# FangjinhuaWang/PatchmatchNet

Measured on AMD Instinct MI355X. Metric: depth-maps/sec at 1600x1200 N=5 src views, higher is better.
Workload: dtype f32

## Files before the change

patchmatchnet_amd/csrc/aggregate.hip:

```cpp
#include <cstring>

#include "pmn_common.hpp"
#define PMN_DIV_DM1(acc, D) ((acc) / (float)((D) - 1))

struct AggArgs {
    const float* cost;
    const float* depth;
    const float* xnorm;
    const float* fweight;
    const float* offsets;
    float* score;
    float* depth_out;
    int K, is_inverse, B, D, h, w;
    float interval_scale;
    int table[2 * PMN_MAX_NEIGHBORS];
};

template <int KMAX, int DL>
__global__ __launch_bounds__(PMN_BLOCK, (KMAX <= 9 ? 3 : 1)) void aggregate_regress_kernel(const AggArgs a) {
#pragma clang fp contract(off)
    constexpr int NPX = PMN_BLOCK / DL;
    __shared__ float red[DL][NPX];
    __shared__ float red2[DL][NPX];
    const int h = a.h, w = a.w, hw = h * w, D = a.D, K = a.K;
// ... 73 lines not shown

    float acc = 0.0f;
#pragma unroll 1
    for (int d = dl; d < D; d += DL) {
        if (ok) {
            const size_t o = ((size_t)b * D + d) * hw + p;
            const float prob = expf((a.score[o] - smax) - lse);
            a.score[o] = prob;
            acc = acc + (a.is_inverse ? (float)d : a.depth[o]) * prob;
        }
    }
    red2[dl][px] = acc;
    __syncthreads();
    if (dl != 0 || !ok) return;
    acc = 0.0f;
#pragma unroll
    for (int i = 0; i < DL; ++i) acc = acc + red2[i][px];
    float out = acc;
    if (a.is_inverse) {
        const float inv_min = 1.0f / a.depth[((size_t)b * D + (D - 1)) * hw + p];
        const float inv_max = 1.0f / a.depth[((size_t)b * D) * hw + p];
        const float inv = inv_max + PMN_DIV_DM1(acc, D) * (inv_min - inv_max);
        out = 1.0f / inv;
    }
    a.depth_out[(size_t)b * hw + p] = out;
}

__device__ __forceinline__ float sigmoid_rcp(float x) {
    const float d = 1.0f + __builtin_amdgcn_exp2f(x * -1.4426950408889634f);
    float r = __builtin_amdgcn_rcpf(d);
    return r * fmaf(-d, r, 2.0f);
}

template <int G, int SL>
__device__ __forceinline__ int agg_group_bcast_i(int v) {
    static_assert(G == 2 || G == 4 || G == 8 || G == 16, "lane groups inside a DPP row");
    if constexpr (G == 2) {
        return __builtin_amdgcn_mov_dpp(v, SL | (SL << 2) | ((2 + SL) << 4) | ((2 + SL) << 6), 0xF, 0xF, true);
    } else if constexpr (G == 4) {
        return __builtin_amdgcn_mov_dpp(v, SL | (SL << 2) | (SL << 4) | (SL << 6), 0xF, 0xF, true);
    } else if constexpr (G == 16) {
        return __builtin_amdgcn_mov_dpp(v, 0x150 + SL, 0xF, 0xF, true);
    } else {
        const int lo = __builtin_amdgcn_update_dpp(v, v, 0x150 + SL, 0xF, 0x3, false);
        return __builtin_amdgcn_update_dpp(lo, v, 0x150 + 8 + SL, 0xF, 0xC, false);
    }
}
template <int G, int SL>
__device__ __forceinline__ float agg_group_bcast_f(float v) {
    return __int_as_float(agg_group_bcast_i<G, SL>(__float_as_int(v)));
}

template <int KMAX>
__device__ __forceinline__ void agg_form_tap_set(const AggArgs& a, int b, int k, int p, int x, int y, int& off, float& w00, float& w01,
                                                 float& w10, float& w11, float& fw) {
    const int h = a.h, w = a.w, hw = h * w, K = a.K;
    const float ox = a.offsets[((size_t)b * 2 * K + 2 * k) * hw + p];
    const float oy = a.offsets[((size_t)b * 2 * K + 2 * k + 1) * hw + p];
    float ix, iy;
    pmn_neighbor_position((float)x, (float)y, a.table[2 * k], a.table[2 * k + 1], ox, oy, h, w, ix, iy);
    const PmnTaps t = pmn_make_taps(ix, iy, h, w);
    off = t.off;
    w00 = t.w00;
    w01 = t.w01;
    w10 = t.w10;
    w11 = t.w11;
    fw = a.fweight[((size_t)b * K + k) * hw + p];
}

template <int KMAX, int DQT>
__global__ __launch_bounds__(PMN_BLOCK, (KMAX <= 9 ? 3 : 1)) void aggregate_regress_q4_kernel(const AggArgs a) {
#pragma clang fp contract(off)
    __shared__ float red[PMN_BLOCK];
    const int h = a.h, w = a.w, hw = h * w, D = a.D, K = a.K, DQ = DQT > 0 ? DQT : D >> 2;
    const int npx = blockDim.x / DQ;
    const int px = threadIdx.x / DQ, q = threadIdx.x - px * DQ;
    const int p_raw = blockIdx.x * npx + px;
    const bool ok = p_raw < hw;
    const int p = ok ? p_raw : hw - 1;
    const int b = blockIdx.y;
    const int y = p / w, x = p - y * w;

    int off[KMAX];
    float w00[KMAX], w01[KMAX], w10[KMAX], w11[KMAX], fw[KMAX];
    if constexpr (DQT > 1) {
        constexpr int KPT = (KMAX + DQT - 1) / DQT;
        int moff[KPT];
        float m00[KPT], m01[KPT], m10[KPT], m11[KPT], mfw[KPT];
#pragma unroll
        for (int i = 0; i < KPT; ++i) {
            const int k = q + i * DQT;
            moff[i] = 0;
            m00[i] = m01[i] = m10[i] = m11[i] = mfw[i] = 0.0f;
            if (k < K) agg_form_tap_set<KMAX>(a, b, k, p, x, y, moff[i], m00[i], m01[i], m10[i], m11[i], mfw[i]);
        }
#define AGG_TAKE(k_)                                                                                         \
    if constexpr ((k_) < KMAX) {                                                                               \
        constexpr int sl_ = (k_) % DQT, it_ = (k_) / DQT;                                                      \
        off[k_] = agg_group_bcast_i<DQT, sl_>(moff[it_]);                                                      \
        w00[k_] = agg_group_bcast_f<DQT, sl_>(m00[it_]);                                                       \
        w01[k_] = agg_group_bcast_f<DQT, sl_>(m01[it_]);                                                       \
        w10[k_] = agg_group_bcast_f<DQT, sl_>(m10[it_]);                                                       \
        w11[k_] = agg_group_bcast_f<DQT, sl_>(m11[it_]);                                                       \
        fw[k_] = agg_group_bcast_f<DQT, sl_>(mfw[it_]);                                                        \
    }
        AGG_TAKE(0) AGG_TAKE(1) AGG_TAKE(2) AGG_TAKE(3) AGG_TAKE(4) AGG_TAKE(5) AGG_TAKE(6) AGG_TAKE(7) AGG_TAKE(8)
        static_assert(KMAX <= 9, "AGG_TAKE list");
#undef AGG_TAKE
    } else {
#pragma unroll
        for (int k = 0; k < KMAX; ++k) {
            off[k] = 0;
            w00[k] = w01[k] = w10[k] = w11[k] = fw[k] = 0.0f;
            if (k < K) agg_form_tap_set<KMAX>(a, b, k, p, x, y, off[k], w00[k], w01[k], w10[k], w11[k], fw[k]);
        }
    }

    const float inv_interval = 1.0f / a.interval_scale;
    const float* xn = a.xnorm + (size_t)b * hw * D + 4 * q;
    const float* cs = a.cost + (size_t)b * hw * D + 4 * q;
    const float4 xc4 = *reinterpret_cast<const float4*>(xn + (size_t)p * D);
    const float xc[4] = {xc4.x, xc4.y, xc4.z, xc4.w};
    float wk[KMAX][4], ck[KMAX][4], wsum[4] = {0.f, 0.f, 0.f, 0.f};
#pragma unroll
    for (int k = 0; k < KMAX; ++k) {
#pragma unroll
        for (int j = 0; j < 4; ++j) wk[k][j] = ck[k][j] = 0.0f;
        if (k < K) {
            const size_t o = (size_t)off[k] * D, o2 = o + (size_t)w * D;
            const float4 xa = *reinterpret_cast<const float4*>(xn + o), xb = *reinterpret_cast<const float4*>(xn + o + D);
            const float4 xcn = *reinterpret_cast<const float4*>(xn + o2), xd = *reinterpret_cast<const float4*>(xn + o2 + D);
            const float4 ca = *reinterpret_cast<const float4*>(cs + o), cb = *reinterpret_cast<const float4*>(cs + o + D);
            const float4 cc = *reinterpret_cast<const float4*>(cs + o2), cd = *reinterpret_cast<const float4*>(cs + o2 + D);
            const float x00[4] = {xa.x, xa.y, xa.z, xa.w}, x01[4] = {xb.x, xb.y, xb.z, xb.w};
            const float x10[4] = {xcn.x, xcn.y, xcn.z, xcn.w}, x11[4] = {xd.x, xd.y, xd.z, xd.w};
            const float c00[4] = {ca.x, ca.y, ca.z, ca.w}, c01[4] = {cb.x, cb.y, cb.z, cb.w};
            const float c10[4] = {cc.x, cc.y, cc.z, cc.w}, c11[4] = {cd.x, cd.y, cd.z, cd.w};
#pragma unroll
            for (int j = 0; j < 4; ++j) {
                const float x1 = fmaf(x11[j], w11[k], fmaf(x10[j], w10[k], fmaf(x01[j], w01[k], x00[j] * w00[k])));
                ck[k][j] = fmaf(c11[j], w11[k], fmaf(c10[j], w10[k], fmaf(c01[j], w01[k], c00[j] * w00[k])));
                float t = fabsf(x1 - xc[j]) * inv_interval;
                t = fminf(fmaxf(t, 0.0f), 4.0f);
                wk[k][j] = sigmoid_rcp(4.0f - 2.0f * t) * fw[k];
                wsum[j] = wsum[j] + wk[k][j];
            }
        }
    }
    float s[4] = {0.f, 0.f, 0.f, 0.f}, rsum[4];
#pragma unroll
    for (int j = 0; j < 4; ++j) rsum[j] = 1.0f / wsum[j];
#pragma unroll
    for (int k = 0; k < KMAX; ++k)
        if (k < K) {
#pragma unroll
            for (int j = 0; j < 4; ++j) s[j] = s[j] + ck[k][j] * (wk[k][j] * rsum[j]);
        }

    float smax = fmaxf(fmaxf(s[0], s[1]), fmaxf(s[2], s[3]));
    red[threadIdx.x] = smax;
    __syncthreads();
    for (int i = 0; i < DQ; ++i) smax = fmaxf(smax, red[px * DQ + i]);
    __syncthreads();
    float esum = ((expf(s[0] - smax) + expf(s[1] - smax)) + expf(s[2] - smax)) + expf(s[3] - smax);
    red[threadIdx.x] = esum;
    __syncthreads();
    esum = 0.0f;
    for (int i = 0; i < DQ; ++i) esum = esum + red[px * DQ + i];
    __syncthreads();
    const float lse = logf(esum);
    float acc = 0.0f;
#pragma unroll
    for (int j = 0; j < 4; ++j) {
        const int d = 4 * q + j;
        const size_t o = ((size_t)b * D + d) * hw + p;
        const float prob = expf((s[j] - smax) - lse);
        if (ok) a.score[o] = prob;
        acc = acc + (a.is_inverse ? (float)d : a.depth[o]) * prob;
    }
    red[threadIdx.x] = acc;
    __syncthreads();
    if (q != 0 || !ok) return;
    acc = 0.0f;
    for (int i = 0; i < DQ; ++i) acc = acc + red[px * DQ + i];
    float out = acc;
    if (a.is_inverse) {
        const float inv_min = 1.0f / a.depth[((size_t)b * D + (D - 1)) * hw + p];
        const float inv_max = 1.0f / a.depth[((size_t)b * D) * hw + p];
        const float inv = inv_max + PMN_DIV_DM1(acc, D) * (inv_min - inv_max);
        out = 1.0f / inv;
    }
    a.depth_out[(size_t)b * hw + p] = out;
}

template <int KMAX>
static int launch_agg_q4(const AggArgs& a, hipStream_t s) {
    const int DQ = a.D / 4, npx = PMN_BLOCK / DQ;
    const dim3 grid((a.h * a.w + npx - 1) / npx, a.B), block(npx * DQ);
    if (DQ == 2) PMN_LAUNCH((aggregate_regress_q4_kernel<KMAX, 2>), grid, block, 0, s, a);
    else if (DQ == 4) PMN_LAUNCH((aggregate_regress_q4_kernel<KMAX, 4>), grid, block, 0, s, a);
    else if (DQ == 8) PMN_LAUNCH((aggregate_regress_q4_kernel<KMAX, 8>), grid, block, 0, s, a);
    else if (DQ == 16) PMN_LAUNCH((aggregate_regress_q4_kernel<KMAX, 16>), grid, block, 0, s, a);
    else PMN_LAUNCH((aggregate_regress_q4_kernel<KMAX, 0>), grid, block, 0, s, a);
    PMN_CHECK_LAUNCH();
    return PMN_OK;
}

template <int KMAX, int DL>
static int launch_agg_dl(const AggArgs& a, hipStream_t s) {
    constexpr int NPX = PMN_BLOCK / DL;
    const dim3 grid((a.h * a.w + NPX - 1) / NPX, a.B), block(PMN_BLOCK);
    PMN_LAUNCH((aggregate_regress_kernel<KMAX, DL>), grid, block, 0, s, a);
    PMN_CHECK_LAUNCH();
    return PMN_OK;
}

template <int KMAX>
static int launch_agg(const AggArgs& a, hipStream_t s) {
    if constexpr (KMAX <= 9) {
        if (a.D % 4 == 0) return launch_agg_q4<KMAX>(a, s);
    }
    if (a.D >= 32) return launch_agg_dl<KMAX, 16>(a, s);
    if (a.D >= 16) return launch_agg_dl<KMAX, 4>(a, s);
    return launch_agg_dl<KMAX, 1>(a, s);
}

extern "C" int pmn_aggregate_regress(const float* cost, const float* depth_sample, const float* xnorm,
                                     const float* feature_weight, const float* eval_offsets, const int* eval_table_host,
                                     int K, float interval_scale, int is_inverse, int B, int D, int h, int w,
                                     float* score_out, float* depth_out, void* stream) {
    if (!cost || !depth_sample || !xnorm || !feature_weight || !eval_offsets || !eval_table_host || !score_out ||
        !depth_out)
        return PMN_ERR_ARG;
    if (B < 1 || D < 1 || h < 2 || w < 2) return PMN_ERR_ARG;
    if (K < 1 || K > PMN_MAX_NEIGHBORS || D > PMN_MAX_DEPTH) return PMN_ERR_SHAPE;
    if (is_inverse && D < 2) return PMN_ERR_ARG;
    AggArgs a;
    memset(&a, 0, sizeof(a));
    a.cost = cost;
    a.depth = depth_sample;
    a.xnorm = xnorm;
    a.fweight = feature_weight;
    a.offsets = eval_offsets;
    a.score = score_out;
    a.depth_out = depth_out;
    a.K = K;
    a.is_inverse = is_inverse;
    a.B = B; a.D = D; a.h = h; a.w = w;
    a.interval_scale = interval_scale;
    for (int i = 0; i < 2 * K; ++i) a.table[i] = eval_table_host[i];
    if (K <= 9) return launch_agg<9>(a, (hipStream_t)stream);
    return launch_agg<17>(a, (hipStream_t)stream);
}
```

patchmatchnet_amd/csrc/hypotheses.hip:

```cpp
#include <cstring>

#include "pmn_common.hpp"
#define PMN_DIV48(u) ((u) / 48.0f)
#define PMN_DIV48R(u) pmn_div_by((u), 48.0f, r48)

struct HypArgs {
    const float* noise;
    const float* depth;
    const float* depth_min;
    const float* depth_max;
    const float* offsets;
    float* depth_sample;
    float* xnorm;
    int depth_shift, num_sample, K, B, h, w;
    float interval_scale;
    int table[2 * PMN_MAX_NEIGHBORS];
};

__device__ __forceinline__ float centre_hypothesis(const HypArgs& a, int b, int qy, int qx, float inv_min, float inv_max,
                                                   float interval, int kc) {
#pragma clang fp contract(off)
    const int h = a.h, w = a.w;
    if (a.noise) {
        const float u = a.noise[((size_t)b * 48 + 24) * h * w + (size_t)qy * w + qx] + 24.0f;
// ... 79 lines not shown
#pragma unroll
        for (int kk = 2; kk <= NP2; kk <<= 1) {
#pragma unroll
            for (int jj = kk >> 1; jj > 0; jj >>= 1) {
#pragma unroll
                for (int i = 0; i < NP2; ++i) {
                    const int l = i ^ jj;
                    if (l > i) {
                        const float lo = fminf(v[i], v[l]), hi = fmaxf(v[i], v[l]);
                        if ((i & kk) == 0) {
                            v[i] = lo;
                            v[l] = hi;
                        } else {
                            v[i] = hi;
                            v[l] = lo;
                        }
                    }
                }
            }
        }
    }

    const float range = inv_min - inv_max;
#pragma unroll
    for (int j = 0; j < NP2; ++j) {
        if (j < D) {
            const size_t o = ((size_t)b * D + j) * hw + p;
            a.depth_sample[o] = v[j];
            a.xnorm[((size_t)b * hw + p) * D + j] = (1.0f / v[j] - inv_max) / range;
        }
    }
}

template <int NP2, int D0T, int KT>
__global__ __launch_bounds__(PMN_BLOCK) void init_hypotheses_fixed_kernel(const HypArgs a) {
#pragma clang fp contract(off)
    static_assert(D0T + KT <= NP2, "hypotheses fit the sorting network");
    const int h = a.h, w = a.w, hw = h * w;
    const int p = blockIdx.x * blockDim.x + threadIdx.x;
    const int b = blockIdx.y;
    if (p >= hw) return;
    const int y = p / w, x = p - y * w;
    const float inv_min = 1.0f / a.depth_min[b];
    const float inv_max = 1.0f / a.depth_max[b];
    constexpr int D = D0T + KT;
    const float interval = (inv_min - inv_max) * a.interval_scale;
    const int k0 = -((a.num_sample + 1) / 2);
    const int kc = k0 + a.num_sample / 2;
    const bool from_noise = a.noise != nullptr;
    const float r48 = pmn_uniform(pmn_rcp_refined(48.0f));

    float v[NP2];
#pragma unroll
    for (int j = 0; j < NP2; ++j) v[j] = __builtin_inff();

    const int ws = w >> a.depth_shift;
    if (from_noise) {
        float u[D0T];
#pragma unroll
        for (int j = 0; j < D0T; ++j) u[j] = a.noise[((size_t)b * 48 + j) * hw + p];
#pragma unroll
        for (int j = 0; j < D0T; ++j) {
            const float inv = inv_max + PMN_DIV48R(u[j] + (float)j) * (inv_min - inv_max);
            v[j] = pmn_div(1.0f, inv);
        }
    } else {
        const float dprev =
            a.depth[(size_t)b * (h >> a.depth_shift) * ws + (size_t)(y >> a.depth_shift) * ws + (x >> a.depth_shift)];
        if (D0T == 1) {
            v[0] = dprev;
        } else {
            const float inv_prev = pmn_div(1.0f, dprev);
#pragma unroll
            for (int j = 0; j < D0T; ++j) {
                float inv = inv_prev + interval * (float)(k0 + j);
                inv = fminf(fmaxf(inv, inv_max), inv_min);
                v[j] = pmn_div(1.0f, inv);
            }
        }
    }

    if constexpr (KT > 0) {
        constexpr int KB = KT < 8 ? KT : 8;
        static_assert(KT % KB == 0, "whole batches");
        const float* cbase = from_noise ? a.noise + ((size_t)b * 48 + 24) * hw
                                        : a.depth + (size_t)b * (h >> a.depth_shift) * ws;
        const int sh = from_noise ? 0 : a.depth_shift, cw = from_noise ? w : ws;
#pragma unroll
        for (int k0b = 0; k0b < KT; k0b += KB) {
            float ox[KB], oy[KB];
#pragma unroll
            for (int i = 0; i < KB; ++i) {
                ox[i] = a.offsets[((size_t)b * 2 * KT + 2 * (k0b + i)) * hw + p];
                oy[i] = a.offsets[((size_t)b * 2 * KT + 2 * (k0b + i) + 1) * hw + p];
            }
            PmnTaps t[KB];
            float c[KB][4];
#pragma unroll
            for (int i = 0; i < KB; ++i) {
                float ix, iy;
                pmn_neighbor_position((float)x, (float)y, a.table[2 * (k0b + i)], a.table[2 * (k0b + i) + 1], ox[i], oy[i], h, w, ix,
                                      iy);
                t[i] = pmn_make_taps(ix, iy, h, w);
                const int qy = t[i].off / w, qx = t[i].off - qy * w;
                c[i][0] = cbase[(size_t)(qy >> sh) * cw + (qx >> sh)];
                c[i][1] = cbase[(size_t)(qy >> sh) * cw + ((qx + 1) >> sh)];
                c[i][2] = cbase[(size_t)((qy + 1) >> sh) * cw + (qx >> sh)];
                c[i][3] = cbase[(size_t)((qy + 1) >> sh) * cw + ((qx + 1) >> sh)];
            }
#pragma unroll
            for (int i = 0; i < KB; ++i) {
                float cc[4];
#pragma unroll
                for (int q = 0; q < 4; ++q) {
                    if (from_noise) {
                        const float inv = inv_max + PMN_DIV48R(c[i][q] + 24.0f) * (inv_min - inv_max);
                        cc[q] = pmn_div(1.0f, inv);
                    } else if (a.num_sample == 1) {
                        cc[q] = c[i][q];
                    } else {
                        float inv = pmn_div(1.0f, c[i][q]) + interval * (float)kc;
                        inv = fminf(fmaxf(inv, inv_max), inv_min);
                        cc[q] = pmn_div(1.0f, inv);
                    }
                }
                v[D0T + k0b + i] = fmaf(cc[3], t[i].w11, fmaf(cc[2], t[i].w10, fmaf(cc[1], t[i].w01, cc[0] * t[i].w00)));
            }
        }
#pragma unroll
        for (int kk = 2; kk <= NP2; kk <<= 1) {
#pragma unroll
            for (int jj = kk >> 1; jj > 0; jj >>= 1) {
#pragma unroll
                for (int i = 0; i < NP2; ++i) {
                    const int l = i ^ jj;
                    if (l > i) {
                        const float lo = fminf(v[i], v[l]), hi = fmaxf(v[i], v[l]);
                        if ((i & kk) == 0) {
                            v[i] = lo;
                            v[l] = hi;
                        } else {
                            v[i] = hi;
                            v[l] = lo;
                        }
                    }
                }
            }
        }
    }

    const float range = inv_min - inv_max, rrange = pmn_rcp_refined(range);
#pragma unroll
    for (int j = 0; j < D; ++j) {
        const size_t o = ((size_t)b * D + j) * hw + p;
        a.depth_sample[o] = v[j];
        a.xnorm[((size_t)b * hw + p) * D + j] = pmn_div_by(pmn_div(1.0f, v[j]) - inv_max, range, rrange);
    }
}

extern "C" int pmn_init_hypotheses(const float* noise, const float* depth, int depth_shift, const float* depth_min,
                                   const float* depth_max, int num_sample, float interval_scale,
                                   const float* propa_offsets, const int* propa_table_host, int K, int B, int h, int w,
                                   float* depth_sample, float* xnorm, void* stream) {
    if ((!noise && !depth) || !depth_min || !depth_max || !depth_sample || !xnorm) return PMN_ERR_ARG;
    if (B < 1 || h < 2 || w < 2 || K < 0 || depth_shift < 0 || depth_shift > 1) return PMN_ERR_ARG;
    if (K > 0 && (!propa_offsets || !propa_table_host)) return PMN_ERR_ARG;
    if (K > 16) return PMN_ERR_SHAPE;
    if (!noise && num_sample < 1) return PMN_ERR_ARG;
    if (depth_shift && ((h | w) & 1)) return PMN_ERR_ARG;
    const int D0 = noise ? 48 : num_sample;
    const int D = D0 + K;
    if (D > PMN_MAX_DEPTH) return PMN_ERR_SHAPE;
    HypArgs a;
    memset(&a, 0, sizeof(a));
    a.noise = noise;
    a.depth = noise ? nullptr : depth;
    a.depth_min = depth_min;
    a.depth_max = depth_max;
    a.offsets = propa_offsets;
    a.depth_sample = depth_sample;
    a.xnorm = xnorm;
    a.depth_shift = depth_shift;
    a.num_sample = noise ? 48 : num_sample;
    a.K = K;
    a.B = B; a.h = h; a.w = w;
    a.interval_scale = interval_scale;
    for (int i = 0; i < 2 * K; ++i) a.table[i] = propa_table_host[i];
    const int bs = (h * w <= 64 * 1024) ? 64 : PMN_BLOCK;
    const dim3 grid((h * w + bs - 1) / bs, B), block(bs);
    hipStream_t s = (hipStream_t)stream;
    if (noise && K == 16) PMN_LAUNCH((init_hypotheses_fixed_kernel<64, 48, 16>), grid, block, 0, s, a);
    else if (!noise && num_sample == 16 && K == 16) PMN_LAUNCH((init_hypotheses_fixed_kernel<32, 16, 16>), grid, block, 0, s, a);
    else if (!noise && num_sample == 8 && K == 8) PMN_LAUNCH((init_hypotheses_fixed_kernel<16, 8, 8>), grid, block, 0, s, a);
    else if (!noise && num_sample == 8 && K == 0) PMN_LAUNCH((init_hypotheses_fixed_kernel<8, 8, 0>), grid, block, 0, s, a);
    else if (D <= 8) PMN_LAUNCH(init_hypotheses_kernel<8>, grid, block, 0, s, a);
    else if (D <= 16) PMN_LAUNCH(init_hypotheses_kernel<16>, grid, block, 0, s, a);
    else if (D <= 32) PMN_LAUNCH(init_hypotheses_kernel<32>, grid, block, 0, s, a);
    else PMN_LAUNCH(init_hypotheses_kernel<64>, grid, block, 0, s, a);
    PMN_CHECK_LAUNCH();
    return PMN_OK;
}
```

patchmatchnet_amd/csrc/pmn_common.hpp:

```cpp
#pragma once
#include <hip/hip_runtime.h>
#include <stdint.h>

#include "../../include/pmn_hip.h"

#define PMN_BLOCK 256

__device__ __forceinline__ float pmn_sigmoid(float x) { return 1.0f / (1.0f + expf(-x)); }

__device__ __forceinline__ float pmn_settle(float v) {
#ifndef PMN_NO_SETTLE
    asm volatile("" : "+v"(v));
#endif
    return v;
}
__device__ __forceinline__ float4 pmn_settle4(float4 v) {
    return make_float4(pmn_settle(v.x), pmn_settle(v.y), pmn_settle(v.z), pmn_settle(v.w));
}

struct PmnTaps {
    int off;
    float w00, w01, w10, w11;
};

__device__ __forceinline__ void pmn_axis(float pos, int size, int& i0c, float& wa, float& wb) {
#pragma clang fp contract(off)
    float f0 = floorf(pos);
    float f1 = f0 + 1.0f;
    float w_lo = f1 - pos;
    float w_hi = pos - f0;
    int i0 = (int)fminf(fmaxf(f0, -2.0f), (float)size);
    i0c = min(max(i0, 0), size - 2);
    wa = 0.0f;
    wb = 0.0f;
    if (i0 == i0c) {
        wa = w_lo;
        wb = w_hi;
    } else if (i0 == -1) {
        wa = w_hi;
    } else if (i0 == size - 1) {
        wb = w_lo;
    }
}

__device__ __forceinline__ PmnTaps pmn_make_taps(float ix, float iy, int hs, int ws) {
#pragma clang fp contract(off)
    int x0c, y0c;
    float ax, bx, ay, by;
    pmn_axis(ix, ws, x0c, ax, bx);
    pmn_axis(iy, hs, y0c, ay, by);
// ... 179 lines not shown
```

patchmatchnet_amd/ops.py:

```python
from __future__ import annotations

import ctypes
from typing import List, Optional, Sequence, Tuple

import numpy as np
import torch

from . import _lib
from ._lib import PmnError, check


_TIMING = None
_TIMING_ON = True


def enable_kernel_timing() -> None:
    global _TIMING, _TIMING_ON
    _TIMING, _TIMING_ON = [], True


def pause_kernel_timing(paused: bool) -> None:
    global _TIMING_ON
    _TIMING_ON = not paused

# ... 260 lines not shown
    dev = ref_nhwc.device
    sim_p = _mlp_dev(similarity_mlp, "similarity_mlp").data_ptr()
    pix_p, vw_out, argmax = None, None, None
    if view_weights is not None:
        _dev(view_weights, "view_weights")
        if tuple(view_weights.shape) != (B, N, h >> vw_shift, w >> vw_shift):
            raise PmnError("Patchmatch Evaluation: Different number of images and view weights")
    else:
        if pixelwise_mlp is None:
            raise PmnError("warp_correlate: pixelwise_mlp required when view_weights is None")
        pix_p = _mlp_dev(pixelwise_mlp, "pixelwise_mlp").data_ptr()
        vw_out = torch.empty((B, N, h, w), dtype=torch.float32, device=dev)
        if want_argmax:
            argmax = torch.empty((B, N, h, w), dtype=torch.int32, device=dev)
    cost = torch.empty((B, h, w, D), dtype=torch.float32, device=dev).permute(0, 3, 1, 2)
    sim = torch.empty((B, G, D, h, w), dtype=torch.float32, device=dev) if want_similarity else None
    with torch.cuda.device(dev):
        if _TIMING is not None and _TIMING_ON:
            ev0, ev1 = torch.cuda.Event(enable_timing=True), torch.cuda.Event(enable_timing=True)
            ev0.record()
        fn = _lib.lib().pmn_warp_correlate if table is None else _lib.lib().pmn_warp_correlate_views
        check(fn(ref_nhwc.data_ptr(), (src_nhwc if table is None else table.table).data_ptr(), rel_proj.data_ptr(),
                 depth_sample.data_ptr(), _ptr(view_weights), vw_shift, sim_p, pix_p, B, N, C,
                 G, D, h, w, hs, ws, cost.data_ptr(), _ptr(vw_out), _ptr(argmax), _ptr(sim),
                 _stream(cost)), "pmn_warp_correlate")
        if _TIMING is not None and _TIMING_ON:
            ev1.record()
            _TIMING.append((ev0, ev1, 4 * B * h * w * ((1 + N) * C + D + N + G * D),
                            f"C{C}_D{D}_{h}x{w}_N{N}_{'vw' if view_weights is not None else 'pixelwise'}"))
    return cost, (view_weights if view_weights is not None else vw_out), argmax, sim


def aggregate_regress(cost: torch.Tensor, depth_sample: torch.Tensor, xnorm: torch.Tensor, feature_weight_: torch.Tensor,
                      eval_offsets: torch.Tensor, table: np.ndarray, interval_scale: float, is_inverse: bool
                      ) -> Tuple[torch.Tensor, torch.Tensor]:
    for n, t in (("depth_sample", depth_sample), ("feature_weight", feature_weight_), ("eval_offsets", eval_offsets)):
        _dev(t, n)
    cost, xnorm = _dlast(cost, "cost"), _dlast(xnorm, "xnorm")
    B, D, h, w = cost.shape
    K = feature_weight_.shape[1]
    if tuple(depth_sample.shape) != (B, D, h, w) or tuple(xnorm.shape) != (B, D, h, w) or \
            tuple(feature_weight_.shape) != (B, K, h, w) or tuple(eval_offsets.shape) != (B, 2 * K, h, w):
        raise PmnError("aggregate_regress: inconsistent shapes")
    tab, tab_p = _host_i32(table, 2 * K, "table")
    score = torch.empty((B, D, h, w), dtype=torch.float32, device=cost.device)
    depth = torch.empty((B, h, w), dtype=torch.float32, device=cost.device)
    with torch.cuda.device(cost.device):
        check(_lib.lib().pmn_aggregate_regress(cost.data_ptr(), depth_sample.data_ptr(), xnorm.data_ptr(),
                                               feature_weight_.data_ptr(), eval_offsets.data_ptr(), tab_p, K,
                                               float(interval_scale), 1 if is_inverse else 0, B, D, h, w,
                                               score.data_ptr(), depth.data_ptr(), _stream(cost)),
              "pmn_aggregate_regress")
    return score, depth


def confidence(score: torch.Tensor, H: int, W: int, want_index: bool = False):
    _dev(score, "score")
    B, D, h, w = score.shape
    conf = torch.empty((B, H, W), dtype=torch.float32, device=score.device)
    idx = torch.empty((B, h, w), dtype=torch.int32, device=score.device) if want_index else None
    with torch.cuda.device(score.device):
        check(_lib.lib().pmn_confidence(score.data_ptr(), B, D, h, w, H, W, conf.data_ptr(), _ptr(idx), _stream(score)),
              "pmn_confidence")
    return conf, idx


def relative_projection(src_projs: Sequence[torch.Tensor], ref_proj: torch.Tensor) -> torch.Tensor:
    inv = torch.inverse(ref_proj)
    return torch.matmul(torch.stack(list(src_projs), dim=1), inv.unsqueeze(1)).contiguous()


def differentiable_warping(src_fea: torch.Tensor, src_proj: torch.Tensor, ref_proj: torch.Tensor,
                           depth_samples: torch.Tensor) -> torch.Tensor:
    src_fea = _dev(src_fea.contiguous(), "src_fea")
    depth_samples = _dev(depth_samples.contiguous(), "depth_samples")
    B, C, hs, ws = src_fea.shape
    _, D, h, w = depth_samples.shape
    proj = torch.matmul(src_proj, torch.inverse(ref_proj)).contiguous()
    _dev(proj, "proj")
    out = torch.empty((B, C, D, h, w), dtype=torch.float32, device=src_fea.device)
    with torch.cuda.device(src_fea.device):
        check(_lib.lib().pmn_differentiable_warping(src_fea.data_ptr(), proj.data_ptr(), depth_samples.data_ptr(), B, C,
                                                    D, h, w, hs, ws, out.data_ptr(), _stream(out)),
              "pmn_differentiable_warping")
# ... 829 lines not shown
```

patchmatchnet_amd/patchmatch.py:

```python
from __future__ import annotations

from typing import List, Optional, Tuple

import numpy as np
import torch
import torch.nn as nn

import warnings

from . import _lib, ops, params
from ._lib import PmnError
from .module import ConvBnReLU3D, is_empty


class _PointwiseMLP(nn.Module):

    _last = "similarity"

    def __init__(self, G: int) -> None:
        super().__init__()
        self.G = G
        self.conv0 = ConvBnReLU3D(in_channels=G, out_channels=16, kernel_size=1, stride=1, pad=0)
        self.conv1 = ConvBnReLU3D(in_channels=16, out_channels=8, kernel_size=1, stride=1, pad=0)
        self._packed: Optional[np.ndarray] = None
# ... 83 lines not shown
        self.pixel_wise_net = PixelwiseNet(self.G)
        self.softmax = nn.LogSoftmax(dim=1)
        self.similarity_net = SimilarityNet(self.G)

    def forward(self, ref_feature: torch.Tensor, src_features: List[torch.Tensor], ref_proj: torch.Tensor,
                src_projs: List[torch.Tensor], depth_sample: torch.Tensor, grid: Optional[torch.Tensor],
                weight: Optional[torch.Tensor], view_weights: torch.Tensor, is_inverse: bool, *,
                fused: Optional[dict] = None, debug: Optional[dict] = None) -> Tuple[torch.Tensor, torch.Tensor, torch.Tensor]:
        N = len(src_features) if src_features is not None else fused["src_nhwc"].shape[0]
        if src_features is not None and src_projs is not None and len(src_features) != len(src_projs):
            raise AssertionError("Patchmatch Evaluation: Different number of images and projection matrices")
        have_vw = not is_empty(view_weights)
        if have_vw and view_weights.size()[1] != N:
            raise AssertionError("Patchmatch Evaluation: Different number of images and view weights")
        f = fused or {}
        ref_nhwc = f.get("ref_nhwc")
        src_nhwc = f.get("src_nhwc")
        rel_proj = f.get("rel_proj")
        if ref_nhwc is None:
            ref_nhwc = ops.nchw_to_nhwc(ref_feature.detach())
        if rel_proj is None:
            rel_proj = ops.relative_projection(src_projs, ref_proj)
        if src_nhwc is None:
            src_nhwc, sizes = ops.stack_sources_padded([s.detach() for s in src_features])
            rel_proj = ops.rescale_projection_rows(rel_proj, sizes, tuple(src_nhwc.shape[2:4]))
        depth_sample = depth_sample.contiguous()
        cost, vw, argmax, sim = ops.warp_correlate(
            ref_nhwc, src_nhwc, rel_proj.contiguous(), depth_sample, view_weights.contiguous() if have_vw else None,
            int(f.get("vw_shift", 0)), self.similarity_net.packed_device(),
            None if have_vw else self.pixel_wise_net.packed_device(), self.G,
            want_similarity=debug is not None, want_argmax=debug is not None and not have_vw)
        if fused is not None and grid is None:
            score, depth = ops.aggregate_regress(cost, depth_sample, f["xnorm"], f["feature_weight"], f["eval_offsets"],
                                                 f["table"], f["interval_scale"], is_inverse)
        else:
            if grid is None or weight is None:
                raise PmnError("Evaluation.forward needs grid and weight (reference signature) or the fused-form arguments")
            B, D, h, w = depth_sample.shape
            K = grid.shape[1] // h
            sampled = torch.nn.functional.grid_sample(cost.contiguous(), grid, mode="bilinear", padding_mode="border",
                                                      align_corners=False).view(B, D, K, h, w)
            score = torch.sum(sampled * weight, dim=2)
            score = torch.exp(self.softmax(score))
            if is_inverse:
                index = torch.arange(0, D, 1, device=score.device).view(1, D, 1, 1)
                index = torch.sum(index * score, dim=1)
                inv_min = 1.0 / depth_sample[:, -1, :, :]
                inv_max = 1.0 / depth_sample[:, 0, :, :]
                depth = 1.0 / (inv_max + index / (D - 1) * (inv_min - inv_max))
            else:
                depth = torch.sum(depth_sample * score, dim=1)
        if debug is not None:
            debug.update(cost=cost, similarity=sim, view_weight_argmax=argmax)
        return depth, score, vw.detach()


class PatchMatch(nn.Module):

    def __init__(self, propagation_out_range: int = 2, patchmatch_iteration: int = 2, patchmatch_num_sample: int = 16,
                 patchmatch_interval_scale: float = 0.025, num_feature: int = 64, G: int = 8,
                 propagate_neighbors: int = 16, evaluate_neighbors: int = 9, stage: int = 3) -> None:
        super().__init__()
        self.patchmatch_iteration = patchmatch_iteration
        self.patchmatch_interval_scale = patchmatch_interval_scale
        self.propa_num_feature = num_feature
        self.G = G
        self.stage = stage
# ... 88 lines not shown
        if rel_proj is None:
            rel_proj = ops.relative_projection(src_projs, ref_proj)
        if src_nhwc is None:
            src_nhwc, sizes = ops.stack_sources_padded([f.detach() for f in src_features])
            rel_proj = ops.rescale_projection_rows(rel_proj, sizes, tuple(src_nhwc.shape[2:4]))
        rel_proj = rel_proj.contiguous()
        depth_min = depth_min.float().contiguous()
        depth_max = depth_max.float().contiguous()

        feature_weight = self.feature_weight_net(ref_nhwc, eval_offsets, self._etable)

        depth_sample = depth
        cur_shift = depth_shift
        score = torch.empty(0, device=device)
        depth_samples: List[torch.Tensor] = []
        for it in range(1, self.patchmatch_iteration + 1):
            is_inverse = self.stage == 1 and it == self.patchmatch_iteration
            first_random = is_empty(depth_sample)
            if first_random and noise is None:
                noise = torch.rand(size=(batch, 48, height, width), device=device)
            propagate = self.propagate_neighbors > 0 and not (self.stage == 1 and it == self.patchmatch_iteration)
            hyp, xnorm = ops.init_hypotheses(
                noise.contiguous() if first_random else None,
                None if first_random else depth_sample.detach().contiguous(), cur_shift, depth_min, depth_max,
                self.depth_initialization.patchmatch_num_sample, self.patchmatch_interval_scale,
                propa_offsets if propagate else None, self._ptable if propagate else None, height, width)
            rec = {} if debug is not None else None
            had_view_weights = not is_empty(view_weights)
            d, score, view_weights = self.evaluation(
                ref_feature=ref_feature, src_features=src_features, ref_proj=ref_proj, src_projs=src_projs, depth_sample=hyp,
                grid=None, weight=None, view_weights=view_weights, is_inverse=is_inverse,
                fused=dict(xnorm=xnorm, eval_offsets=eval_offsets, table=self._etable, feature_weight=feature_weight,
                           interval_scale=self.patchmatch_interval_scale, vw_shift=vw_shift, ref_nhwc=ref_nhwc,
                           src_nhwc=src_nhwc, rel_proj=rel_proj), debug=rec)
            if not had_view_weights:
                vw_shift = 0
            if rec is not None:
                rec.update(depth_sample=hyp, xnorm=xnorm, feature_weight=feature_weight, score=score, depth=d,
                           view_weights=view_weights, eval_offsets=eval_offsets, propa_offsets=propa_offsets)
                debug.append(rec)
            depth_sample = d.unsqueeze(1)
            cur_shift = 0
            depth_samples.append(depth_sample)
        return depth_samples, score, view_weights
```

Before: 399.4.

## Split hypothesis init across lanes, DPP softmax reductions, skip unused score writes

```diff
diff --git a/patchmatchnet_amd/csrc/aggregate.hip b/patchmatchnet_amd/csrc/aggregate.hip
--- a/patchmatchnet_amd/csrc/aggregate.hip
+++ b/patchmatchnet_amd/csrc/aggregate.hip
@@ -129,25 +129,6 @@
     return r * fmaf(-d, r, 2.0f);
 }
 
-template <int G, int SL>
-__device__ __forceinline__ int agg_group_bcast_i(int v) {
-    static_assert(G == 2 || G == 4 || G == 8 || G == 16, "lane groups inside a DPP row");
-    if constexpr (G == 2) {
-        return __builtin_amdgcn_mov_dpp(v, SL | (SL << 2) | ((2 + SL) << 4) | ((2 + SL) << 6), 0xF, 0xF, true);
-    } else if constexpr (G == 4) {
-        return __builtin_amdgcn_mov_dpp(v, SL | (SL << 2) | (SL << 4) | (SL << 6), 0xF, 0xF, true);
-    } else if constexpr (G == 16) {
-        return __builtin_amdgcn_mov_dpp(v, 0x150 + SL, 0xF, 0xF, true);
-    } else {
-        const int lo = __builtin_amdgcn_update_dpp(v, v, 0x150 + SL, 0xF, 0x3, false);
-        return __builtin_amdgcn_update_dpp(lo, v, 0x150 + 8 + SL, 0xF, 0xC, false);
-    }
-}
-template <int G, int SL>
-__device__ __forceinline__ float agg_group_bcast_f(float v) {
-    return __int_as_float(agg_group_bcast_i<G, SL>(__float_as_int(v)));
-}
-
 template <int KMAX>
 __device__ __forceinline__ void agg_form_tap_set(const AggArgs& a, int b, int k, int p, int x, int y, int& off, float& w00, float& w01,
                                                  float& w10, float& w11, float& fw) {
@@ -165,11 +146,22 @@
     fw = a.fweight[((size_t)b * K + k) * hw + p];
 }
 
+template <int G, int I = 0>
+__device__ __forceinline__ float agg_group_max(float v, float acc) {
+    if constexpr (I == G) return acc;
+    else return agg_group_max<G, I + 1>(v, fmaxf(acc, pmn_group_bcast_f<G, I>(v)));
+}
+template <int G, int I = 0>
+__device__ __forceinline__ float agg_group_sum(float v, float acc = 0.0f) {
+#pragma clang fp contract(off)
+    if constexpr (I == G) return acc;
+    else return agg_group_sum<G, I + 1>(v, acc + pmn_group_bcast_f<G, I>(v));
+}
+
 template <int KMAX, int DQT>
 __global__ __launch_bounds__(PMN_BLOCK, (KMAX <= 9 ? 3 : 1)) void aggregate_regress_q4_kernel(const AggArgs a) {
 #pragma clang fp contract(off)
-    __shared__ float red[PMN_BLOCK];
-    const int h = a.h, w = a.w, hw = h * w, D = a.D, K = a.K, DQ = DQT > 0 ? DQT : D >> 2;
+    const int h = a.h, w = a.w, hw = h * w, D = DQT > 0 ? 4 * DQT : a.D, K = a.K, DQ = DQT > 0 ? DQT : D >> 2;
     const int npx = blockDim.x / DQ;
     const int px = threadIdx.x / DQ, q = threadIdx.x - px * DQ;
     const int p_raw = blockIdx.x * npx + px;
@@ -194,12 +186,12 @@
 #define AGG_TAKE(k_)                                                                                         \
     if constexpr ((k_) < KMAX) {                                                                               \
         constexpr int sl_ = (k_) % DQT, it_ = (k_) / DQT;                                                      \
-        off[k_] = agg_group_bcast_i<DQT, sl_>(moff[it_]);                                                      \
-        w00[k_] = agg_group_bcast_f<DQT, sl_>(m00[it_]);                                                       \
-        w01[k_] = agg_group_bcast_f<DQT, sl_>(m01[it_]);                                                       \
-        w10[k_] = agg_group_bcast_f<DQT, sl_>(m10[it_]);                                                       \
-        w11[k_] = agg_group_bcast_f<DQT, sl_>(m11[it_]);                                                       \
-        fw[k_] = agg_group_bcast_f<DQT, sl_>(mfw[it_]);                                                        \
+        off[k_] = pmn_group_bcast_i<DQT, sl_>(moff[it_]);                                                      \
+        w00[k_] = pmn_group_bcast_f<DQT, sl_>(m00[it_]);                                                       \
+        w01[k_] = pmn_group_bcast_f<DQT, sl_>(m01[it_]);                                                       \
+        w10[k_] = pmn_group_bcast_f<DQT, sl_>(m10[it_]);                                                       \
+        w11[k_] = pmn_group_bcast_f<DQT, sl_>(m11[it_]);                                                       \
+        fw[k_] = pmn_group_bcast_f<DQT, sl_>(mfw[it_]);                                                        \
     }
         AGG_TAKE(0) AGG_TAKE(1) AGG_TAKE(2) AGG_TAKE(3) AGG_TAKE(4) AGG_TAKE(5) AGG_TAKE(6) AGG_TAKE(7) AGG_TAKE(8)
         static_assert(KMAX <= 9, "AGG_TAKE list");
@@ -254,32 +246,46 @@
             for (int j = 0; j < 4; ++j) s[j] = s[j] + ck[k][j] * (wk[k][j] * rsum[j]);
         }
 
+    __shared__ float red[DQT > 1 ? 1 : PMN_BLOCK];
     float smax = fmaxf(fmaxf(s[0], s[1]), fmaxf(s[2], s[3]));
-    red[threadIdx.x] = smax;
-    __syncthreads();
-    for (int i = 0; i < DQ; ++i) smax = fmaxf(smax, red[px * DQ + i]);
-    __syncthreads();
+    if constexpr (DQT > 1) {
+        smax = pmn_settle(agg_group_max<DQT>(smax, smax));
+    } else {
+        red[threadIdx.x] = smax;
+        __syncthreads();
+        for (int i = 0; i < DQ; ++i) smax = fmaxf(smax, red[px * DQ + i]);
+        __syncthreads();
+    }
     float esum = ((expf(s[0] - smax) + expf(s[1] - smax)) + expf(s[2] - smax)) + expf(s[3] - smax);
-    red[threadIdx.x] = esum;
-    __syncthreads();
-    esum = 0.0f;
-    for (int i = 0; i < DQ; ++i) esum = esum + red[px * DQ + i];
-    __syncthreads();
-    const float lse = logf(esum);
+    if constexpr (DQT > 1) {
+        esum = agg_group_sum<DQT>(esum);
+    } else {
+        red[threadIdx.x] = esum;
+        __syncthreads();
+        esum = 0.0f;
+        for (int i = 0; i < DQ; ++i) esum = esum + red[px * DQ + i];
+        __syncthreads();
+    }
+    const float lse = pmn_settle(logf(esum));
     float acc = 0.0f;
 #pragma unroll
     for (int j = 0; j < 4; ++j) {
         const int d = 4 * q + j;
         const size_t o = ((size_t)b * D + d) * hw + p;
         const float prob = expf((s[j] - smax) - lse);
-        if (ok) a.score[o] = prob;
+        if (ok && a.score) a.score[o] = prob;
         acc = acc + (a.is_inverse ? (float)d : a.depth[o]) * prob;
     }
-    red[threadIdx.x] = acc;
-    __syncthreads();
-    if (q != 0 || !ok) return;
-    acc = 0.0f;
-    for (int i = 0; i < DQ; ++i) acc = acc + red[px * DQ + i];
+    if constexpr (DQT > 1) {
+        acc = agg_group_sum<DQT>(acc);
+        if (q != 0 || !ok) return;
+    } else {
+        red[threadIdx.x] = acc;
+        __syncthreads();
+        if (q != 0 || !ok) return;
+        acc = 0.0f;
+        for (int i = 0; i < DQ; ++i) acc = acc + red[px * DQ + i];
+    }
     float out = acc;
     if (a.is_inverse) {
         const float inv_min = 1.0f / a.depth[((size_t)b * D + (D - 1)) * hw + p];
@@ -326,9 +332,8 @@
                                      const float* feature_weight, const float* eval_offsets, const int* eval_table_host,
                                      int K, float interval_scale, int is_inverse, int B, int D, int h, int w,
                                      float* score_out, float* depth_out, void* stream) {
-    if (!cost || !depth_sample || !xnorm || !feature_weight || !eval_offsets || !eval_table_host || !score_out ||
-        !depth_out)
-        return PMN_ERR_ARG;
+    if (!cost || !depth_sample || !xnorm || !feature_weight || !eval_offsets || !eval_table_host || !depth_out) return PMN_ERR_ARG;
+    if (!score_out && !(K <= 9 && D % 4 == 0)) return PMN_ERR_ARG;
     if (B < 1 || D < 1 || h < 2 || w < 2) return PMN_ERR_ARG;
     if (K < 1 || K > PMN_MAX_NEIGHBORS || D > PMN_MAX_DEPTH) return PMN_ERR_SHAPE;
     if (is_inverse && D < 2) return PMN_ERR_ARG;
diff --git a/patchmatchnet_amd/csrc/hypotheses.hip b/patchmatchnet_amd/csrc/hypotheses.hip
--- a/patchmatchnet_amd/csrc/hypotheses.hip
+++ b/patchmatchnet_amd/csrc/hypotheses.hip
@@ -135,129 +135,201 @@
     }
 }
 
+#ifndef PMN_HYP_LANES_SORT
+#define PMN_HYP_LANES_SORT 4
+#endif
+#ifndef PMN_HYP_LANES_PLAIN
+#define PMN_HYP_LANES_PLAIN 2
+#endif
+template <int D0T, int KT>
+constexpr int hyp_lanes() {
+    return KT > 0 ? PMN_HYP_LANES_SORT : PMN_HYP_LANES_PLAIN;
+}
+
+template <int N, int O, int NV>
+__device__ __forceinline__ void hyp_sort_network(float (&v)[NV]) {
+#pragma unroll
+    for (int kk = 2; kk <= N; kk <<= 1) {
+#pragma unroll
+        for (int jj = kk >> 1; jj > 0; jj >>= 1) {
+#pragma unroll
+            for (int i = 0; i < N; ++i) {
+                const int l = i ^ jj;
+                if (l > i) {
+                    const float lo = fminf(v[O + i], v[O + l]), hi = fmaxf(v[O + i], v[O + l]);
+                    if ((i & kk) == 0) {
+                        v[O + i] = lo;
+                        v[O + l] = hi;
+                    } else {
+                        v[O + i] = hi;
+                        v[O + l] = lo;
+                    }
+                }
+            }
+        }
+    }
+}
+
+template <int N>
+__device__ __forceinline__ void hyp_merge_network(float (&v)[N]) {
+#pragma unroll
+    for (int jj = N >> 1; jj > 0; jj >>= 1) {
+#pragma unroll
+        for (int i = 0; i < N; ++i) {
+            const int l = i ^ jj;
+            if (l > i) {
+                const float lo = fminf(v[i], v[l]), hi = fmaxf(v[i], v[l]);
+                v[i] = lo;
+                v[l] = hi;
+            }
+        }
+    }
+}
+
+template <int L, int N, int S, int NV>
+__device__ __forceinline__ void hyp_all_gather(const float (&mine)[N], float (&v)[NV], int base) {
+    if constexpr (S < L) {
+#pragma unroll
+        for (int i = 0; i < N; ++i) v[base + S * N + i] = pmn_group_bcast_f<L, S>(mine[i]);
+        hyp_all_gather<L, N, S + 1>(mine, v, base);
+    }
+}
+
 template <int NP2, int D0T, int KT>
 __global__ __launch_bounds__(PMN_BLOCK) void init_hypotheses_fixed_kernel(const HypArgs a) {
 #pragma clang fp contract(off)
-    static_assert(D0T + KT <= NP2, "hypotheses fit the sorting network");
+    constexpr int D = D0T + KT, L = hyp_lanes<D0T, KT>();
+    constexpr int OWN = D0T / L, NB = KT / L, NQ = D / (4 * L);
+    static_assert(D == NP2, "the merge needs no padding");
+    static_assert(D0T >= 2 && D0T % L == 0 && KT % L == 0 && D % (4 * L) == 0, "whole shares per lane");
+    static_assert(KT > 0 || OWN == 4, "without propagation a lane stores the quad it formed");
     const int h = a.h, w = a.w, hw = h * w;
-    const int p = blockIdx.x * blockDim.x + threadIdx.x;
+    const int tid = blockIdx.x * blockDim.x + threadIdx.x;
+    const int p = tid / L, g = tid - p * L;
     const int b = blockIdx.y;
     if (p >= hw) return;
     const int y = p / w, x = p - y * w;
     const float inv_min = 1.0f / a.depth_min[b];
     const float inv_max = 1.0f / a.depth_max[b];
-    constexpr int D = D0T + KT;
     const float interval = (inv_min - inv_max) * a.interval_scale;
     const int k0 = -((a.num_sample + 1) / 2);
     const int kc = k0 + a.num_sample / 2;
     const bool from_noise = a.noise != nullptr;
     const float r48 = pmn_uniform(pmn_rcp_refined(48.0f));
 
-    float v[NP2];
-#pragma unroll
-    for (int j = 0; j < NP2; ++j) v[j] = __builtin_inff();
-
+    float mine[OWN];
     const int ws = w >> a.depth_shift;
     if (from_noise) {
-        float u[D0T];
-#pragma unroll
-        for (int j = 0; j < D0T; ++j) u[j] = a.noise[((size_t)b * 48 + j) * hw + p];
-#pragma unroll
-        for (int j = 0; j < D0T; ++j) {
-            const float inv = inv_max + PMN_DIV48R(u[j] + (float)j) * (inv_min - inv_max);
-            v[j] = pmn_div(1.0f, inv);
+        float u[OWN];
+#pragma unroll
+        for (int i = 0; i < OWN; ++i) u[i] = a.noise[((size_t)b * 48 + (g * OWN + i)) * hw + p];
+#pragma unroll
+        for (int i = 0; i < OWN; ++i) {
+            const float inv = inv_max + PMN_DIV48R(u[i] + (float)(g * OWN + i)) * (inv_min - inv_max);
+            mine[i] = pmn_div(1.0f, inv);
         }
     } else {
         const float dprev =
             a.depth[(size_t)b * (h >> a.depth_shift) * ws + (size_t)(y >> a.depth_shift) * ws + (x >> a.depth_shift)];
-        if (D0T == 1) {
-            v[0] = dprev;
-        } else {
-            const float inv_prev = pmn_div(1.0f, dprev);
-#pragma unroll
-            for (int j = 0; j < D0T; ++j) {
-                float inv = inv_prev + interval * (float)(k0 + j);
-                inv = fminf(fmaxf(inv, inv_max), inv_min);
-                v[j] = pmn_div(1.0f, inv);
-            }
-        }
-    }
-
+        const float inv_prev = pmn_div(1.0f, dprev);
+#pragma unroll
+        for (int i = 0; i < OWN; ++i) {
+            float inv = inv_prev + interval * (float)(k0 + g * OWN + i);
+            inv = fminf(fmaxf(inv, inv_max), inv_min);
+            mine[i] = pmn_div(1.0f, inv);
+        }
+    }
+
+    float out[NQ][4];
     if constexpr (KT > 0) {
-        constexpr int KB = KT < 8 ? KT : 8;
-        static_assert(KT % KB == 0, "whole batches");
         const float* cbase = from_noise ? a.noise + ((size_t)b * 48 + 24) * hw
                                         : a.depth + (size_t)b * (h >> a.depth_shift) * ws;
         const int sh = from_noise ? 0 : a.depth_shift, cw = from_noise ? w : ws;
-#pragma unroll
-        for (int k0b = 0; k0b < KT; k0b += KB) {
-            float ox[KB], oy[KB];
-#pragma unroll
-            for (int i = 0; i < KB; ++i) {
-                ox[i] = a.offsets[((size_t)b * 2 * KT + 2 * (k0b + i)) * hw + p];
-                oy[i] = a.offsets[((size_t)b * 2 * KT + 2 * (k0b + i) + 1) * hw + p];
-            }
-            PmnTaps t[KB];
-            float c[KB][4];
-#pragma unroll
-            for (int i = 0; i < KB; ++i) {
-                float ix, iy;
-                pmn_neighbor_position((float)x, (float)y, a.table[2 * (k0b + i)], a.table[2 * (k0b + i) + 1], ox[i], oy[i], h, w, ix,
-                                      iy);
-                t[i] = pmn_make_taps(ix, iy, h, w);
-                const int qy = t[i].off / w, qx = t[i].off - qy * w;
-                c[i][0] = cbase[(size_t)(qy >> sh) * cw + (qx >> sh)];
-                c[i][1] = cbase[(size_t)(qy >> sh) * cw + ((qx + 1) >> sh)];
-                c[i][2] = cbase[(size_t)((qy + 1) >> sh) * cw + (qx >> sh)];
-                c[i][3] = cbase[(size_t)((qy + 1) >> sh) * cw + ((qx + 1) >> sh)];
-            }
-#pragma unroll
-            for (int i = 0; i < KB; ++i) {
-                float cc[4];
-#pragma unroll
-                for (int q = 0; q < 4; ++q) {
-                    if (from_noise) {
-                        const float inv = inv_max + PMN_DIV48R(c[i][q] + 24.0f) * (inv_min - inv_max);
-                        cc[q] = pmn_div(1.0f, inv);
-                    } else if (a.num_sample == 1) {
-                        cc[q] = c[i][q];
-                    } else {
-                        float inv = pmn_div(1.0f, c[i][q]) + interval * (float)kc;
-                        inv = fminf(fmaxf(inv, inv_max), inv_min);
-                        cc[q] = pmn_div(1.0f, inv);
-                    }
-                }
-                v[D0T + k0b + i] = fmaf(cc[3], t[i].w11, fmaf(cc[2], t[i].w10, fmaf(cc[1], t[i].w01, cc[0] * t[i].w00)));
-            }
-        }
-#pragma unroll
-        for (int kk = 2; kk <= NP2; kk <<= 1) {
-#pragma unroll
-            for (int jj = kk >> 1; jj > 0; jj >>= 1) {
-#pragma unroll
-                for (int i = 0; i < NP2; ++i) {
-                    const int l = i ^ jj;
-                    if (l > i) {
-                        const float lo = fminf(v[i], v[l]), hi = fmaxf(v[i], v[l]);
-                        if ((i & kk) == 0) {
-                            v[i] = lo;
-                            v[l] = hi;
-                        } else {
-                            v[i] = hi;
-                            v[l] = lo;
-                        }
-                    }
-                }
-            }
-        }
+        float ox[NB], oy[NB], prop[NB];
+#pragma unroll
+        for (int i = 0; i < NB; ++i) {
+            ox[i] = a.offsets[((size_t)b * 2 * KT + 2 * (g * NB + i)) * hw + p];
+            oy[i] = a.offsets[((size_t)b * 2 * KT + 2 * (g * NB + i) + 1) * hw + p];
+        }
+        PmnTaps t[NB];
+        float c[NB][4];
+#pragma unroll
+        for (int i = 0; i < NB; ++i) {
+            int dy = 0, dx = 0;
+#pragma unroll
+            for (int s = 0; s < L; ++s)
+                if (g == s) {
+                    dy = a.table[2 * (s * NB + i)];
+                    dx = a.table[2 * (s * NB + i) + 1];
+                }
+            float ix, iy;
+            pmn_neighbor_position((float)x, (float)y, dy, dx, ox[i], oy[i], h, w, ix, iy);
+            t[i] = pmn_make_taps(ix, iy, h, w);
+            const int qy = t[i].off / w, qx = t[i].off - qy * w;
+            c[i][0] = cbase[(size_t)(qy >> sh) * cw + (qx >> sh)];
+            c[i][1] = cbase[(size_t)(qy >> sh) * cw + ((qx + 1) >> sh)];
+            c[i][2] = cbase[(size_t)((qy + 1) >> sh) * cw + (qx >> sh)];
+            c[i][3] = cbase[(size_t)((qy + 1) >> sh) * cw + ((qx + 1) >> sh)];
+        }
+#pragma unroll
+        for (int i = 0; i < NB; ++i) {
+            float cc[4];
+#pragma unroll
+            for (int q = 0; q < 4; ++q) {
+                if (from_noise) {
+                    const float inv = inv_max + PMN_DIV48R(c[i][q] + 24.0f) * (inv_min - inv_max);
+                    cc[q] = pmn_div(1.0f, inv);
+                } else if (a.num_sample == 1) {
+                    cc[q] = c[i][q];
+                } else {
+                    float inv = pmn_div(1.0f, c[i][q]) + interval * (float)kc;
+                    inv = fminf(fmaxf(inv, inv_max), inv_min);
+                    cc[q] = pmn_div(1.0f, inv);
+                }
+            }
+            prop[i] = fmaf(cc[3], t[i].w11, fmaf(cc[2], t[i].w10, fmaf(cc[1], t[i].w01, cc[0] * t[i].w00)));
+        }
+
+        float v[NP2];
+        hyp_all_gather<L, OWN, 0>(mine, v, 0);
+        hyp_all_gather<L, NB, 0>(prop, v, D0T);
+
+        bool bitonic = true;
+#pragma unroll
+        for (int j = 0; j + 1 < D0T; ++j) bitonic = bitonic && (v[j] >= v[j + 1]);
+#pragma unroll
+        for (int j = D0T - 1; j < D; ++j) bitonic = bitonic && (v[j] == v[j]);
+        if (__builtin_expect(bitonic, 1)) {
+            hyp_sort_network<KT, D0T>(v);
+            hyp_merge_network<NP2>(v);
+        } else {
+            hyp_sort_network<NP2, 0>(v);
+        }
+#pragma unroll
+        for (int m = 0; m < NQ; ++m)
+#pragma unroll
+            for (int q = 0; q < 4; ++q) {
+                out[m][q] = v[4 * L * m + q];
+#pragma unroll
+                for (int s = 1; s < L; ++s)
+                    if (g == s) out[m][q] = v[4 * (s + L * m) + q];
+            }
+    } else {
+#pragma unroll
+        for (int q = 0; q < 4; ++q) out[0][q] = mine[q];
     }
 
     const float range = inv_min - inv_max, rrange = pmn_rcp_refined(range);
 #pragma unroll
-    for (int j = 0; j < D; ++j) {
-        const size_t o = ((size_t)b * D + j) * hw + p;
-        a.depth_sample[o] = v[j];
-        a.xnorm[((size_t)b * hw + p) * D + j] = pmn_div_by(pmn_div(1.0f, v[j]) - inv_max, range, rrange);
+    for (int m = 0; m < NQ; ++m) {
+        const int j0 = 4 * (g + L * m);
+        float xn[4];
+#pragma unroll
+        for (int q = 0; q < 4; ++q) {
+            a.depth_sample[((size_t)b * D + j0 + q) * hw + p] = out[m][q];
+            xn[q] = pmn_div_by(pmn_div(1.0f, out[m][q]) - inv_max, range, rrange);
+        }
+        *reinterpret_cast<float4*>(a.xnorm + ((size_t)b * hw + p) * D + j0) = make_float4(xn[0], xn[1], xn[2], xn[3]);
     }
 }
 
@@ -271,6 +343,7 @@
     if (K > 16) return PMN_ERR_SHAPE;
     if (!noise && num_sample < 1) return PMN_ERR_ARG;
     if (depth_shift && ((h | w) & 1)) return PMN_ERR_ARG;
+    if ((uintptr_t)xnorm & 15) return PMN_ERR_ARG;
     const int D0 = noise ? 48 : num_sample;
     const int D = D0 + K;
     if (D > PMN_MAX_DEPTH) return PMN_ERR_SHAPE;
@@ -291,11 +364,15 @@
     for (int i = 0; i < 2 * K; ++i) a.table[i] = propa_table_host[i];
     const int bs = (h * w <= 64 * 1024) ? 64 : PMN_BLOCK;
     const dim3 grid((h * w + bs - 1) / bs, B), block(bs);
+    auto lane_grid = [&](int lanes) { return dim3((unsigned)(((long long)h * w * lanes + bs - 1) / bs), B); };
     hipStream_t s = (hipStream_t)stream;
-    if (noise && K == 16) PMN_LAUNCH((init_hypotheses_fixed_kernel<64, 48, 16>), grid, block, 0, s, a);
-    else if (!noise && num_sample == 16 && K == 16) PMN_LAUNCH((init_hypotheses_fixed_kernel<32, 16, 16>), grid, block, 0, s, a);
-    else if (!noise && num_sample == 8 && K == 8) PMN_LAUNCH((init_hypotheses_fixed_kernel<16, 8, 8>), grid, block, 0, s, a);
-    else if (!noise && num_sample == 8 && K == 0) PMN_LAUNCH((init_hypotheses_fixed_kernel<8, 8, 0>), grid, block, 0, s, a);
+    if (noise && K == 16) PMN_LAUNCH((init_hypotheses_fixed_kernel<64, 48, 16>), lane_grid(hyp_lanes<48, 16>()), block, 0, s, a);
+    else if (!noise && num_sample == 16 && K == 16)
+        PMN_LAUNCH((init_hypotheses_fixed_kernel<32, 16, 16>), lane_grid(hyp_lanes<16, 16>()), block, 0, s, a);
+    else if (!noise && num_sample == 8 && K == 8)
+        PMN_LAUNCH((init_hypotheses_fixed_kernel<16, 8, 8>), lane_grid(hyp_lanes<8, 8>()), block, 0, s, a);
+    else if (!noise && num_sample == 8 && K == 0)
+        PMN_LAUNCH((init_hypotheses_fixed_kernel<8, 8, 0>), lane_grid(hyp_lanes<8, 0>()), block, 0, s, a);
     else if (D <= 8) PMN_LAUNCH(init_hypotheses_kernel<8>, grid, block, 0, s, a);
     else if (D <= 16) PMN_LAUNCH(init_hypotheses_kernel<16>, grid, block, 0, s, a);
     else if (D <= 32) PMN_LAUNCH(init_hypotheses_kernel<32>, grid, block, 0, s, a);
diff --git a/patchmatchnet_amd/csrc/pmn_common.hpp b/patchmatchnet_amd/csrc/pmn_common.hpp
--- a/patchmatchnet_amd/csrc/pmn_common.hpp
+++ b/patchmatchnet_amd/csrc/pmn_common.hpp
@@ -16,6 +16,25 @@
 }
 __device__ __forceinline__ float4 pmn_settle4(float4 v) {
     return make_float4(pmn_settle(v.x), pmn_settle(v.y), pmn_settle(v.z), pmn_settle(v.w));
+}
+
+template <int G, int SL>
+__device__ __forceinline__ int pmn_group_bcast_i(int v) {
+    static_assert(G == 2 || G == 4 || G == 8 || G == 16, "lane groups inside a DPP row");
+    if constexpr (G == 2) {
+        return __builtin_amdgcn_mov_dpp(v, SL | (SL << 2) | ((2 + SL) << 4) | ((2 + SL) << 6), 0xF, 0xF, true);
+    } else if constexpr (G == 4) {
+        return __builtin_amdgcn_mov_dpp(v, SL | (SL << 2) | (SL << 4) | (SL << 6), 0xF, 0xF, true);
+    } else if constexpr (G == 16) {
+        return __builtin_amdgcn_mov_dpp(v, 0x150 + SL, 0xF, 0xF, true);
+    } else {
+        const int lo = __builtin_amdgcn_update_dpp(v, v, 0x150 + SL, 0xF, 0x3, false);
+        return __builtin_amdgcn_update_dpp(lo, v, 0x150 + 8 + SL, 0xF, 0xC, false);
+    }
+}
+template <int G, int SL>
+__device__ __forceinline__ float pmn_group_bcast_f(float v) {
+    return __int_as_float(pmn_group_bcast_i<G, SL>(__float_as_int(v)));
 }
 
 struct PmnTaps {
diff --git a/patchmatchnet_amd/ops.py b/patchmatchnet_amd/ops.py
--- a/patchmatchnet_amd/ops.py
+++ b/patchmatchnet_amd/ops.py
@@ -316,8 +316,8 @@
 
 
 def aggregate_regress(cost: torch.Tensor, depth_sample: torch.Tensor, xnorm: torch.Tensor, feature_weight_: torch.Tensor,
-                      eval_offsets: torch.Tensor, table: np.ndarray, interval_scale: float, is_inverse: bool
-                      ) -> Tuple[torch.Tensor, torch.Tensor]:
+                      eval_offsets: torch.Tensor, table: np.ndarray, interval_scale: float, is_inverse: bool,
+                      want_score: bool = True) -> Tuple[Optional[torch.Tensor], torch.Tensor]:
     for n, t in (("depth_sample", depth_sample), ("feature_weight", feature_weight_), ("eval_offsets", eval_offsets)):
         _dev(t, n)
     cost, xnorm = _dlast(cost, "cost"), _dlast(xnorm, "xnorm")
@@ -327,13 +327,14 @@
             tuple(feature_weight_.shape) != (B, K, h, w) or tuple(eval_offsets.shape) != (B, 2 * K, h, w):
         raise PmnError("aggregate_regress: inconsistent shapes")
     tab, tab_p = _host_i32(table, 2 * K, "table")
-    score = torch.empty((B, D, h, w), dtype=torch.float32, device=cost.device)
+    skip_score = not want_score and K <= 9 and D % 4 == 0
+    score = None if skip_score else torch.empty((B, D, h, w), dtype=torch.float32, device=cost.device)
     depth = torch.empty((B, h, w), dtype=torch.float32, device=cost.device)
     with torch.cuda.device(cost.device):
         check(_lib.lib().pmn_aggregate_regress(cost.data_ptr(), depth_sample.data_ptr(), xnorm.data_ptr(),
                                                feature_weight_.data_ptr(), eval_offsets.data_ptr(), tab_p, K,
                                                float(interval_scale), 1 if is_inverse else 0, B, D, h, w,
-                                               score.data_ptr(), depth.data_ptr(), _stream(cost)),
+                                               _ptr(score), depth.data_ptr(), _stream(cost)),
               "pmn_aggregate_regress")
     return score, depth
 
diff --git a/patchmatchnet_amd/patchmatch.py b/patchmatchnet_amd/patchmatch.py
--- a/patchmatchnet_amd/patchmatch.py
+++ b/patchmatchnet_amd/patchmatch.py
@@ -139,7 +139,10 @@
             want_similarity=debug is not None, want_argmax=debug is not None and not have_vw)
         if fused is not None and grid is None:
             score, depth = ops.aggregate_regress(cost, depth_sample, f["xnorm"], f["feature_weight"], f["eval_offsets"],
-                                                 f["table"], f["interval_scale"], is_inverse)
+                                                 f["table"], f["interval_scale"], is_inverse,
+                                                 want_score=bool(f.get("want_score", True)))
+            if score is None:
+                score = torch.empty(0, device=depth.device)
         else:
             if grid is None or weight is None:
                 raise PmnError("Evaluation.forward needs grid and weight (reference signature) or the fused-form arguments")
@@ -294,7 +297,8 @@
                 grid=None, weight=None, view_weights=view_weights, is_inverse=is_inverse,
                 fused=dict(xnorm=xnorm, eval_offsets=eval_offsets, table=self._etable, feature_weight=feature_weight,
                            interval_scale=self.patchmatch_interval_scale, vw_shift=vw_shift, ref_nhwc=ref_nhwc,
-                           src_nhwc=src_nhwc, rel_proj=rel_proj), debug=rec)
+                           src_nhwc=src_nhwc, rel_proj=rel_proj,
+                           want_score=it == self.patchmatch_iteration or debug is not None), debug=rec)
             if not had_view_weights:
                 vw_shift = 0
             if rec is not None:
```

After: 402.2 (median of 3 runs). Within noise of the previous version (+0.7%).
